# bbye98/mdhelper

Hardware: AMD Instinct MI355X
Metric: pair-distances binned/sec (higher is better)
Workload: dtype f32 filter + f64 contract arithmetic, u64 counts

## Files before the change

include/mdx.h:

```cpp
#ifndef MDX_H
#define MDX_H

#include <stddef.h>
#include <stdint.h>

#ifdef __cplusplus
extern "C" {
#endif

#define MDX_VERSION 100

#define MDX_OK 0
#define MDX_ERR_INVALID_VALUE (-1)
#define MDX_ERR_UNSUPPORTED (-2)
#define MDX_ERR_NO_DEVICE (-3)
#define MDX_ERR_HIP (-4)
#define MDX_ERR_ROCFFT (-5)
#define MDX_ERR_RCCL (-6)
#define MDX_ERR_OUT_OF_MEMORY (-7)
#define MDX_ERR_STATE (-8)
#define MDX_ERR_IO (-9)


const char *mdx_last_error(void);
// ... 39 lines not shown
#define MDX_RDF_ALGO_FILTER_F32 2
#define MDX_RDF_ALGO_CELL 3

int mdx_rdf_create(mdx_rdf_t *out, int dev, int n_bins, const double *edges,
                   int64_t excl1, int64_t excl2, int algo);
int mdx_rdf_destroy(mdx_rdf_t h);
int mdx_rdf_reset(mdx_rdf_t h);
int mdx_rdf_accumulate(mdx_rdf_t h, const float *pos1, int64_t n1, const float *pos2,
                       int64_t n2, const float *boxes, int64_t n_frames);
int mdx_rdf_set_drop_axis(mdx_rdf_t h, int axis);
int mdx_rdf_set_grouping(mdx_rdf_t h, int which, int64_t n_groups, const int64_t *offsets,
                         const double *masses);
int mdx_rdf_accumulate_device(mdx_rdf_t h, const float *d_pos1, int64_t n1,
                              const float *d_pos2, int64_t n2, const float *d_boxes,
                              int64_t n_frames);
int mdx_rdf_counts(mdx_rdf_t h, int64_t *counts);
int mdx_rdf_synchronize(mdx_rdf_t h);
int mdx_rdf_allreduce(mdx_rdf_t h, mdx_comm_t comm);
int mdx_rdf_stats(mdx_rdf_t h, int64_t *launches, double *kernel_ms,
                  int64_t *pairs_evaluated, int64_t *pairs_exact, int64_t *pairs_computed);
int mdx_rdf_enable_timing(mdx_rdf_t h, int on);
int mdx_rdf_debug_counters(mdx_rdf_t h, int64_t out[4]);
int mdx_rdf_kernel_clock(mdx_rdf_t h, double *hz);
int mdx_rdf_debug_sorted(mdx_rdf_t h, int64_t frame, int64_t n_pad, float *pw, float *po);

int mdx_radial_histogram(int dev, const float *pos1, int64_t n1, const float *pos2,
                         int64_t n2, int n_bins, const double *edges, const float dims[6],
                         int64_t excl1, int64_t excl2, int64_t *counts);

typedef struct mdx_sq *mdx_sq_t;

int mdx_sq_create(mdx_sq_t *out, int dev, const double *wavevectors, int64_t n_q,
                  const int64_t *group_offsets, int n_groups, const int32_t *pairs,
                  int n_pairs);
int mdx_sq_destroy(mdx_sq_t h);
int mdx_sq_reset(mdx_sq_t h);
int mdx_sq_set_grouping(mdx_sq_t h, int64_t n_molecules, const int64_t *offsets, const double *masses);
int mdx_sq_set_chains(mdx_sq_t h, int64_t chain_length);
int mdx_sq_accumulate(mdx_sq_t h, const float *pos, int64_t n, int64_t n_frames);
int mdx_sq_accumulate_device(mdx_sq_t h, const float *d_pos, int64_t n, int64_t n_frames);
int mdx_sq_synchronize(mdx_sq_t h);
int mdx_sq_result(mdx_sq_t h, double *ssf);
int mdx_sq_allreduce(mdx_sq_t h, mdx_comm_t comm);
int mdx_sq_stats(mdx_sq_t h, int64_t *launches, double *kernel_ms);
int mdx_sq_enable_timing(mdx_sq_t h, int on);
int mdx_fourier_sum(int dev, const double *wavevectors, int64_t n_q, const double *positions,
// ... 195 lines not shown
```

mdhelper_amd/_core.py:

```python

from __future__ import annotations

import ctypes
from ctypes import byref, c_double, c_int, c_int64, c_size_t, c_void_p

import numpy as np

from . import _lib
from ._lib import check, lib


def _ptr(a):
    return None if a is None else a.ctypes.data_as(c_void_p)


class DeviceArray:

    def __init__(self, shape, dtype, dev: int = 0):
        self.shape = tuple(int(s) for s in np.atleast_1d(shape))
        self.dtype = np.dtype(dtype)
        self.dev = dev
        self.nbytes = int(np.prod(self.shape)) * self.dtype.itemsize
        p = c_void_p()
        check(lib().mdx_malloc(dev, self.nbytes, byref(p)))
# ... 235 lines not shown
                                            _ptr(i1), n1, _ptr(i2), n2))

    def counts(self):
        out = np.zeros(self.n_bins, dtype=np.int64)
        check(lib().mdx_rdf_counts(self.handle, _ptr(out)))
        return out

    def synchronize(self):
        check(lib().mdx_rdf_synchronize(self.handle))

    def reset(self):
        check(lib().mdx_rdf_reset(self.handle))

    def allreduce(self, comm: RcclComm):
        check(lib().mdx_rdf_allreduce(self.handle, comm.handle))

    def stats(self):
        n, ms, pe, px, pc = c_int64(), c_double(), c_int64(), c_int64(), c_int64()
        check(lib().mdx_rdf_stats(self.handle, byref(n), byref(ms), byref(pe), byref(px), byref(pc)))
        raw = np.zeros(4, dtype=np.int64)
        check(lib().mdx_rdf_debug_counters(self.handle, _ptr(raw)))
        hz = c_double()
        check(lib().mdx_rdf_kernel_clock(self.handle, byref(hz)))
        return {"launches": n.value, "kernel_ms": ms.value, "pairs_evaluated": pe.value,
                "pairs_exact": px.value, "pairs_computed": pc.value,
                "cell_units": int(raw[1]), "cell_units_general": int(raw[2]),
                "clock_hz": hz.value}


def radial_histogram_device(pos1, pos2, n_bins, edges, dims, exclusion=None, dev=0):
    p1 = np.ascontiguousarray(pos1, dtype=np.float32).reshape(-1, 3)
    p2 = np.ascontiguousarray(pos2, dtype=np.float32).reshape(-1, 3)
    box = None if dims is None else np.ascontiguousarray(dims, dtype=np.float32).reshape(6)
    edges = np.ascontiguousarray(edges, dtype=np.float64)
    e1, e2 = (0, 0) if exclusion is None else (int(exclusion[0]), int(exclusion[1]))
    counts = np.zeros(n_bins, dtype=np.int64)
    same = pos2 is pos1
    check(lib().mdx_radial_histogram(dev, _ptr(p1), p1.shape[0], _ptr(p1 if same else p2),
                                     p2.shape[0], n_bins, _ptr(edges), _ptr(box), e1, e2,
                                     _ptr(counts)))
    return counts


class SqEngine(_Engine):

    _destroy = "mdx_sq_destroy"

    def __init__(self, wavevectors, group_sizes, pairs, *, dev=0, timing=False):
        self.q = np.ascontiguousarray(wavevectors, dtype=np.float64).reshape(-1, 3)
        self.offsets = np.concatenate(([0], np.cumsum(group_sizes))).astype(np.int64)
# ... 809 lines not shown
```

mdhelper_amd/_lib.py:

```python

from __future__ import annotations

import ctypes
import os
import pathlib
from ctypes import POINTER, c_char_p, c_double, c_float, c_int, c_int32, c_int64, c_size_t, c_uint64, c_void_p

_PKG = pathlib.Path(__file__).resolve().parent
LIB_PATH = pathlib.Path(os.environ.get("MDX_LIBRARY", _PKG / "libmdx.so"))

MDX_OK = 0
_EXC = {
    -1: ValueError,
    -2: NotImplementedError,
    -3: RuntimeError,
    -4: RuntimeError,
    -5: RuntimeError,
    -6: RuntimeError,
    -7: MemoryError,
    -8: RuntimeError,
    -9: OSError,
}

RDF_ALGO = {"auto": 0, "exact": 1, "filter": 2, "cell": 3}
# ... 21 lines not shown
    "mdx_synth_random_walk_f64": (c_int, [c_int, _vp, c_int64, c_int64, POINTER(c_float), c_float, c_uint64]),
    "mdx_comm_unique_id": (c_int, [_vp]),
    "mdx_comm_init_rank": (c_int, [POINTER(_vp), c_int, _vp, c_int, c_int]),
    "mdx_comm_destroy": (c_int, [_vp]),
    "mdx_comm_count": (c_int, [_vp, POINTER(c_int), POINTER(c_int), POINTER(c_int)]),
    "mdx_comm_barrier": (c_int, [_vp]),
    "mdx_comm_allreduce_f64": (c_int, [_vp, _vp, c_int64, c_int]),
    "mdx_comm_allreduce_i64": (c_int, [_vp, _vp, c_int64]),
    "mdx_rdf_create": (c_int, [POINTER(_vp), c_int, c_int, _vp, c_int64, c_int64, c_int]),
    "mdx_rdf_destroy": (c_int, [_vp]),
    "mdx_rdf_reset": (c_int, [_vp]),
    "mdx_rdf_accumulate": (c_int, [_vp, _vp, c_int64, _vp, c_int64, _vp, c_int64]),
    "mdx_rdf_accumulate_device": (c_int, [_vp, _vp, c_int64, _vp, c_int64, _vp, c_int64]),
    "mdx_rdf_set_drop_axis": (c_int, [_vp, c_int]),
    "mdx_rdf_set_grouping": (c_int, [_vp, c_int, c_int64, _vp, _vp]),
    "mdx_rdf_counts": (c_int, [_vp, _vp]),
    "mdx_rdf_synchronize": (c_int, [_vp]),
    "mdx_rdf_allreduce": (c_int, [_vp, _vp]),
    "mdx_rdf_stats": (c_int, [_vp, POINTER(c_int64), POINTER(c_double), POINTER(c_int64), POINTER(c_int64),
                              POINTER(c_int64)]),
    "mdx_rdf_enable_timing": (c_int, [_vp, c_int]),
    "mdx_rdf_debug_counters": (c_int, [_vp, _vp]),
    "mdx_rdf_kernel_clock": (c_int, [_vp, POINTER(c_double)]),
    "mdx_rdf_debug_sorted": (c_int, [_vp, c_int64, c_int64, _vp, _vp]),
    "mdx_radial_histogram": (c_int, [c_int, _vp, c_int64, _vp, c_int64, c_int, _vp, _vp, c_int64, c_int64, _vp]),
    "mdx_sq_create": (c_int, [POINTER(_vp), c_int, _vp, c_int64, _vp, c_int, _vp, c_int]),
    "mdx_sq_destroy": (c_int, [_vp]),
    "mdx_sq_reset": (c_int, [_vp]),
    "mdx_sq_accumulate": (c_int, [_vp, _vp, c_int64, c_int64]),
    "mdx_sq_accumulate_device": (c_int, [_vp, _vp, c_int64, c_int64]),
    "mdx_sq_result": (c_int, [_vp, _vp]),
    "mdx_sq_allreduce": (c_int, [_vp, _vp]),
    "mdx_sq_stats": (c_int, [_vp, POINTER(c_int64), POINTER(c_double)]),
    "mdx_sq_enable_timing": (c_int, [_vp, c_int]),
    "mdx_fourier_sum": (c_int, [c_int, _vp, c_int64, _vp, c_int64, _vp]),
    "mdx_isf_create": (c_int, [POINTER(_vp), c_int, _vp, c_int64, _vp, c_int, _vp, c_int, c_int, c_int]),
    "mdx_isf_destroy": (c_int, [_vp]),
    "mdx_isf_reset": (c_int, [_vp]),
    "mdx_isf_accumulate": (c_int, [_vp, _vp, c_int64, c_int64]),
    "mdx_isf_result": (c_int, [_vp, _vp, _vp]),
    "mdx_isf_stats": (c_int, [_vp, POINTER(c_int64), POINTER(c_double), POINTER(c_int64)]),
    "mdx_isf_enable_timing": (c_int, [_vp, c_int]),
    "mdx_msd_create": (c_int, [POINTER(_vp), c_int, c_int64, c_int, c_int]),
    "mdx_msd_destroy": (c_int, [_vp]),
    "mdx_msd_reset": (c_int, [_vp]),
    "mdx_msd_n_fft": (c_int, [_vp, POINTER(c_int64)]),
# ... 235 lines not shown
```

mdhelper_amd/csrc/mdx_rdf.hip:

```cpp

#include "mdx_common.hpp"
#include "mdx_internal.hpp"
#include "mdx_molecules.hpp"
#include "mdx_rdf_device.hpp"
#include "mdx_rdf_cell.hpp"
#include "mdx_traj.hpp"

#include <cmath>

namespace mdx {


static double thresh_ge(double e)
{
    if (!(e > 0.0))
        return 0.0;
    double t = e * e;
    while (std::sqrt(t) >= e && t > 0.0)
        t = std::nextafter(t, 0.0);
    while (std::sqrt(t) < e)
        t = std::nextafter(t, INFINITY);
    return t;
}

static double thresh_gt(double e)
{
    if (e < 0.0)
        return 0.0;
    return thresh_ge(std::nextafter(e, INFINITY));
}
// ... 280 lines not shown
    std::vector<double> edges;
    std::vector<double> thresh;
    double t_lo = 0, t_hi = 0;
    int64_t excl1 = 0, excl2 = 0;
    int algo = MDX_RDF_ALGO_AUTO;
    int n_rep = 32;
    DeviceBuffer d_thresh, d_counts, d_total, d_pack1, d_pack2, d_misc, d_tri;
    DeviceBuffer d_stats;
    DeviceBuffer d_work;
    const void *occ_kernel = nullptr;
    size_t occ_lds = 0;
    int64_t occ_blocks_per_xcd = 1;
    size_t last_offset = 0;
    int64_t last_frames = 0, last_n_pad = 0;
    bool last_lazy = false;
    MoleculeStage grouping[2];
    int drop_axis = -1;
    DeviceBuffer d_drop[2], d_drop_box;
    DeviceBuffer d_stage1[2], d_stage2[2], d_boxes[2], d_index[2];
    DeviceBuffer d_rawslab[2];
    StagePipeline pipe;
    DeviceBuffer d_pw1, d_po1, d_bb1, d_pw2, d_po2, d_bb2;
    DeviceBuffer d_bb16_1, d_bb16_2;
    StreamTimer timer;
    int64_t pairs_evaluated = 0;
    int64_t pairs_bruteforce = 0;
    bool reduced_global = false;
};

static int launch_tiles(mdx_rdf *h, RdfArgs &a, int mode, int ipt, bool pbc, bool excl,
                        int64_t n_frames)
{
    const int T = 256 * ipt;
    size_t base = sizeof(float4) * T + sizeof(double) * (h->n_bins + 1);
    const size_t lds_budget = 64 * 1024;
    int n_hist = 4;
    while (n_hist > 1 && base + size_t(n_hist) * h->n_bins * 4 > lds_budget)
        n_hist >>= 1;
    size_t lds = base + size_t(n_hist) * h->n_bins * 4;
    const bool gh = lds > lds_budget;
    if (gh)
        lds = sizeof(float4) * T;
    a.n_hist = n_hist;
    a.chunk = a.self ? 4 : 8;
    void (*kern)(RdfArgs) = nullptr;
#define MDX_PICK(M, I, P, E) \
// ... 25 lines not shown
        hipLaunchKernelGGL(kern, grid, dim3(256), lds, h->stream, a);
    }
    h->timer.end(ev);
    MDX_HIP(hipGetLastError());
    return MDX_OK;
}

static int accumulate_cell(mdx_rdf *h, const float *d_pos1, int64_t n1, const float *d_pos2,
                           int64_t n2, const float *d_boxes, int64_t n_frames, bool self, bool excl,
                           const float *d_tri = nullptr)
{
    const bool tri = d_tri != nullptr;
    const int64_t n1p = ceil_div(n1, 128) * 128, n2p = ceil_div(n2, 128) * 128;
    constexpr int64_t CHUNK_BOX_BYTES = CELL_CHUNK >= 4 ? 32 / CELL_CHUNK : 0;
    const int64_t per_frame = (32 + 1 + CHUNK_BOX_BYTES) * (n1p + (self ? 0 : n2p));
    const char *slab_env = getenv("MDX_RDF_SLAB_BYTES");
    const int64_t slab_bytes = slab_env ? std::max<int64_t>(1, atoll(slab_env)) : (int64_t(5) << 29);
    int64_t slab = std::max<int64_t>(1, slab_bytes / per_frame);
    slab = std::min<int64_t>(slab, 32768);
    if (slab >= 256)
        slab -= slab % 256;
    slab = std::min<int64_t>(slab, n_frames);
    const bool lazy_orig = !tri && h->excl1 <= 1 && h->excl2 <= 1;
    const size_t e_p1 = size_t(n1p) * slab, e_b1 = size_t(n1p / 64) * 2 * slab;
    const size_t e_c1 = CELL_CHUNK >= 4 ? size_t(n1p / CELL_CHUNK) * 2 * slab : 16;
    const size_t e_p2 = size_t(n2p) * slab, e_b2 = size_t(n2p / 64) * 2 * slab;
    const size_t e_c2 = CELL_CHUNK >= 4 ? size_t(n2p / CELL_CHUNK) * 2 * slab : 16;
    MDX_TRY(h->d_pw1.ensure(16 * e_p1));
    if (!lazy_orig)
        MDX_TRY(h->d_po1.ensure(16 * e_p1));
    MDX_TRY(h->d_bb1.ensure(16 * e_b1));
    MDX_TRY(h->d_bb16_1.ensure(16 * e_c1));
    if (!self) {
        MDX_TRY(h->d_bb16_2.ensure(16 * e_c2));
        MDX_TRY(h->d_pw2.ensure(16 * e_p2));
        if (!lazy_orig)
            MDX_TRY(h->d_po2.ensure(16 * e_p2));
        MDX_TRY(h->d_bb2.ensure(16 * e_b2));
    }
    unsigned *d_misc = h->d_misc.as<unsigned>();
    if (!tri)
        hipLaunchKernelGGL(rdf_check_boxes_kernel, dim3((unsigned)ceil_div(n_frames, 256)), dim3(256),
                           0, h->stream, d_boxes, n_frames, d_misc + 1);

    size_t base = sizeof(float4) * 256 + sizeof(double) * (h->n_bins + 1);
    const size_t lds_budget = 64 * 1024;
    const size_t lds_six_blocks = 13 * 1024;
    int n_hist = 8;
    while (n_hist > 4 && base + size_t(n_hist) * cell_hist_stride(h->n_bins) * 4 > lds_six_blocks)
        n_hist >>= 1;
    while (n_hist > 1 && base + size_t(n_hist) * cell_hist_stride(h->n_bins) * 4 > lds_budget)
        n_hist >>= 1;
    size_t lds = base + size_t(n_hist) * cell_hist_stride(h->n_bins) * 4;
    const bool gh = lds > lds_budget;
    if (gh)
        lds = sizeof(float4) * 256;
    const bool lower = h->edges.front() > 0.0;
    void (*kern)(CellArgs) = nullptr;
#define MDX_CELL_PICK(E, L)                                                                     \
    kern = tri ? (gh ? rdf_cell_pair_kernel<E, L, 1, true> : rdf_cell_pair_kernel<E, L, 0, true>) \
               : (gh ? rdf_cell_pair_kernel<E, L, 1> : rdf_cell_pair_kernel<E, L, 0>)
    if (excl && lower) MDX_CELL_PICK(true, true);
    else if (excl) MDX_CELL_PICK(true, false);
    else if (lower) MDX_CELL_PICK(false, true);
    else MDX_CELL_PICK(false, false);
#undef MDX_CELL_PICK
    if (h->occ_kernel != reinterpret_cast<const void *>(kern) || h->occ_lds != lds) {
        int per_cu = 0, cus = 0;
        MDX_HIP(hipOccupancyMaxActiveBlocksPerMultiprocessor(&per_cu, reinterpret_cast<const void *>(kern), 256, lds));
        MDX_HIP(hipDeviceGetAttribute(&cus, hipDeviceAttributeMultiprocessorCount, h->dev));
        h->occ_kernel = reinterpret_cast<const void *>(kern);
        h->occ_lds = lds;
        h->occ_blocks_per_xcd = std::max<int64_t>(1, int64_t(std::max(per_cu, 1)) * std::max(cus, 8) / 8);
    }
    const int64_t blocks_per_xcd = h->occ_blocks_per_xcd;

    hipStream_t s_sort = h->stream;
    for (int64_t f0 = 0; f0 < n_frames; f0 += slab) {
        const int64_t nf = std::min(slab, n_frames - f0);
        float4 *pw1 = h->d_pw1.as<float4>();
        float4 *po1 = lazy_orig ? nullptr : h->d_po1.as<float4>();
        float4 *bb1 = h->d_bb1.as<float4>(), *bc1 = h->d_bb16_1.as<float4>();
        float4 *pw2 = self ? pw1 : h->d_pw2.as<float4>();
        float4 *po2 = self ? po1 : (lazy_orig ? nullptr : h->d_po2.as<float4>());
        float4 *bb2 = self ? bb1 : h->d_bb2.as<float4>();
        float4 *bc2 = self ? bc1 : h->d_bb16_2.as<float4>();
        unsigned *d_maxabs = d_misc;
        h->last_offset = 0;
        h->last_frames = nf;
        h->last_n_pad = n1p;
        h->last_lazy = lazy_orig;
        {
            auto sort = tri ? rdf_cell_sort_kernel<true> : rdf_cell_sort_kernel<false>;
            const float *cells = tri ? d_tri + f0 * 9 : d_boxes + f0 * 6;
            hipLaunchKernelGGL(sort, dim3((unsigned)nf), dim3(SORT_THREADS), 0, s_sort,
                               d_pos1 + f0 * n1 * 3, cells, (int)n1, (int)n1p, excl ? h->excl1 : 0,
                               pw1, po1, bb1, bc1, d_maxabs);
            if (!self)
                hipLaunchKernelGGL(sort, dim3((unsigned)nf), dim3(SORT_THREADS), 0, s_sort,
                                   d_pos2 + f0 * n2 * 3, cells, (int)n2, (int)n2p,
                                   excl ? h->excl2 : 0, pw2, po2, bb2, bc2, d_maxabs);
        }
        CellArgs a{};
        a.pw1 = pw1;
        a.po1 = po1;
        a.bb1 = bb1;
        a.pw2 = pw2;
        a.po2 = po2;
        a.bb2 = bb2;
        a.bb16_2 = bc2;
        a.in1 = lazy_orig ? d_pos1 + f0 * n1 * 3 : nullptr;
        a.in2 = lazy_orig ? d_pos2 + f0 * n2 * 3 : nullptr;
        a.n1_in = (int)n1;
        a.n2_in = (int)n2;
        a.tags_everywhere = (self && h->excl1 == 1 && h->excl2 == 1) ? 0 : 1;
        a.boxes = tri ? nullptr : d_boxes + f0 * 6;
        a.tri = tri ? d_tri + f0 * 9 : nullptr;
        a.thresh = h->d_thresh.as<double>();
        a.counts = h->d_counts.as<unsigned long long>();
        a.maxabs_bits = d_maxabs;
        a.exact_counter = h->d_stats.as<unsigned long long>();
        a.tilepair_counter = a.exact_counter + 1;
        a.clock_counter = h->timer.enabled ? a.exact_counter + 3 : nullptr;
        a.t_lo = h->t_lo;
        a.t_hi = h->t_hi;
        a.r0 = h->edges.front();
        a.r1 = h->edges.back();
        a.n1p = (int)n1p;
        a.n2p = (int)n2p;
        a.n_bins = h->n_bins;
        a.n_hist = n_hist;
        a.n_rep = h->n_rep;
        a.self = self ? 1 : 0;
        a.work = h->d_work.as<unsigned>();
        {
            const char *fu = getenv("MDX_RDF_LDS_FLUSH_UNITS");
            a.flush_units = fu ? (unsigned)std::min<long long>(std::max<long long>(atoll(fu), 1), 1 << 18) : (1u << 18);
        }
        const int64_t tiles = n1p / 128;
        hipEvent_t ev = h->timer.begin();
        const int64_t launch_frames = std::max<int64_t>(8, std::min<int64_t>(32768, ((int64_t(1) << 30) / tiles) * 8));
        for (int64_t g0 = 0; g0 < nf; g0 += launch_frames) {
            a.frame0 = (int)g0;
            a.n_frames = (int)std::min<int64_t>(launch_frames, nf - g0);
            a.spread = a.n_frames < 8 ? 1 : 0;
            const int64_t items_per_xcd = a.spread ? ceil_div(int64_t(a.n_frames) * tiles, 8)
                                                   : ceil_div(a.n_frames, 8) * tiles;
            const unsigned grid = 8u * (unsigned)std::min<int64_t>(blocks_per_xcd, items_per_xcd);
            MDX_HIP(hipMemsetAsync(h->d_work.ptr, 0, CELL_WORK_BYTES, h->stream));
            hipLaunchKernelGGL(kern, dim3(grid), dim3(256), lds, h->stream, a);
        }
        h->timer.end(ev);
        MDX_HIP(hipGetLastError());
    }
    h->pairs_evaluated += n_frames * n1 * n2;
    return MDX_OK;
}

static int accumulate_ortho(mdx_rdf *h, const float *d_pos1, int64_t n1, const float *d_pos2,
                            int64_t n2, const float *d_boxes, int64_t n_frames)
{
    if (n_frames == 0 || n1 == 0 || n2 == 0)
        return MDX_OK;
    if (h->reduced_global)
        return fail(MDX_ERR_STATE, "handle holds all-reduced counts; call mdx_rdf_reset() first");
    const bool same = (d_pos2 == nullptr || (d_pos2 == d_pos1 && n2 == n1));
    if (d_pos2 == nullptr) {
        d_pos2 = d_pos1;
        n2 = n1;
    }
    const bool excl = h->excl1 > 0;
    const bool self = same && (!excl || h->excl1 == h->excl2);
    MDX_REQUIRE(n1 < (int64_t(1) << 30) && n2 < (int64_t(1) << 30), "too many particles");

    int algo = h->algo;
    if (algo == MDX_RDF_ALGO_AUTO)
        algo = d_boxes ? MDX_RDF_ALGO_CELL : MDX_RDF_ALGO_FILTER_F32;
// ... 389 lines not shown
        if (hipMemcpy(h->d_thresh.ptr, h->thresh.data(), sizeof(double) * (n_bins + 1),
                      hipMemcpyHostToDevice) != hipSuccess) {
            rc = fail(MDX_ERR_HIP, "threshold upload failed");
            break;
        }
    } while (0);
    if (rc != MDX_OK) {
        mdx_rdf_destroy(h);
        return rc;
    }
    *out = h;
    return mdx_rdf_reset(h);
}

int mdx_rdf_destroy(mdx_rdf_t h)
{
    if (!h)
        return MDX_OK;
    (void)hipSetDevice(h->dev);
    if (h->stream)
        (void)hipStreamSynchronize(h->stream);
    if (h->pipe.copy_stream)
        (void)hipStreamSynchronize(h->pipe.copy_stream);
    h->timer.destroy();
    h->pipe.destroy();
    for (DeviceBuffer *b : {&h->d_thresh, &h->d_counts, &h->d_total, &h->d_pack1, &h->d_pack2,
                            &h->d_stage1[0], &h->d_stage2[0], &h->d_boxes[0], &h->d_stage1[1],
                            &h->d_stage2[1], &h->d_boxes[1], &h->d_rawslab[0], &h->d_rawslab[1], &h->d_index[0], &h->d_index[1], &h->d_tri, &h->d_misc, &h->d_stats, &h->d_work, &h->d_pw1,
                            &h->d_po1, &h->d_bb1, &h->d_pw2, &h->d_po2, &h->d_bb2, &h->d_bb16_1,
                            &h->d_bb16_2, &h->d_drop[0], &h->d_drop[1], &h->d_drop_box})
        b->recycle();
    h->grouping[0].recycle();
    h->grouping[1].recycle();
    if (h->stream)
        stream_release(h->stream);
    delete h;
    return MDX_OK;
}

int mdx_rdf_reset(mdx_rdf_t h)
{
    MDX_REQUIRE(h, "NULL handle");
    MDX_TRY(set_device(h->dev));
    MDX_HIP(hipStreamSynchronize(h->stream));
    MDX_HIP(hipMemsetAsync(h->d_counts.ptr, 0, sizeof(uint64_t) * size_t(h->n_rep) * h->n_bins,
                           h->stream));
    MDX_HIP(hipMemsetAsync(h->d_misc.ptr, 0, 64, h->stream));
    MDX_HIP(hipMemsetAsync(h->d_stats.ptr, 0, RDF_STAT_BYTES, h->stream));
    MDX_HIP(hipStreamSynchronize(h->stream));
    h->timer.reset();
    h->pairs_evaluated = 0;
    h->pairs_bruteforce = 0;
    h->reduced_global = false;
    return MDX_OK;
}

int mdx_rdf_set_drop_axis(mdx_rdf_t h, int axis)
{
    MDX_REQUIRE(h, "NULL handle");
    MDX_REQUIRE(axis >= -1 && axis <= 2, "axis must be 0, 1, 2 or -1 (none)");
    h->drop_axis = axis;
    return MDX_OK;
}

int mdx_rdf_set_grouping(mdx_rdf_t h, int which, int64_t n_groups, const int64_t *offsets,
                         const double *masses)
{
    MDX_REQUIRE(h, "NULL handle");
    MDX_REQUIRE(which == 1 || which == 2, "which must be 1 or 2");
    MDX_TRY(set_device(h->dev));
    MDX_HIP(hipStreamSynchronize(h->stream));
    return h->grouping[which - 1].set(n_groups, offsets, masses);
}

int mdx_rdf_accumulate_device(mdx_rdf_t h, const float *d_pos1, int64_t n1, const float *d_pos2,
// ... 153 lines not shown
int mdx_rdf_kernel_clock(mdx_rdf_t h, double *hz)
{
    MDX_REQUIRE(h && hz, "NULL argument");
    MDX_TRY(set_device(h->dev));
    unsigned long long st[5];
    MDX_TRY(read_stats(h, st));
    *hz = st[4] ? double(st[3]) / double(st[4]) * 1.0e8 : 0.0;
    return MDX_OK;
}

int mdx_rdf_debug_counters(mdx_rdf_t h, int64_t out[4])
{
    MDX_REQUIRE(h && out, "NULL argument");
    MDX_TRY(set_device(h->dev));
    unsigned long long raw[5];
    MDX_TRY(read_stats(h, raw));
    out[0] = (int64_t)raw[0];
    out[1] = (int64_t)raw[1];
    out[2] = (int64_t)raw[2];
    out[3] = h->pairs_bruteforce;
    return MDX_OK;
}

int mdx_rdf_debug_sorted(mdx_rdf_t h, int64_t frame, int64_t n_pad, float *pw, float *po)
{
    MDX_REQUIRE(h && pw && po, "NULL argument");
    MDX_TRY(set_device(h->dev));
    MDX_HIP(hipStreamSynchronize(h->stream));
    MDX_REQUIRE(h->last_frames > 0, "no slab has gone through the cell-sorted path yet");
    MDX_REQUIRE(frame >= 0 && frame < h->last_frames, "frame %lld outside the last slab (%lld frames)",
                (long long)frame, (long long)h->last_frames);
    MDX_REQUIRE(n_pad == h->last_n_pad, "n_pad is %lld for the last slab", (long long)h->last_n_pad);
    MDX_HIP(hipMemcpy(pw, h->d_pw1.as<float4>() + h->last_offset + frame * n_pad, size_t(16) * n_pad,
                      hipMemcpyDeviceToHost));
    if (h->last_lazy)
        return fail(MDX_ERR_STATE, "the last slab has no sorted originals (exclusion 0 or 1): pw is filled, "
                    "po is not; MDX_RDF_SORTED_ORIGINALS=1 materialises them");
    MDX_HIP(hipMemcpy(po, h->d_po1.as<float4>() + h->last_offset + frame * n_pad, size_t(16) * n_pad,
                      hipMemcpyDeviceToHost));
    return MDX_OK;
}

int mdx_rdf_enable_timing(mdx_rdf_t h, int on)
{
    MDX_REQUIRE(h, "NULL handle");
    h->timer.enabled = on != 0;
// ... 40 lines not shown
```

mdhelper_amd/csrc/mdx_rdf_cell.hpp:

```cpp
#pragma once

#include "mdx_rdf_device.hpp"

struct CellArgs {
    const float4 *pw1, *po1, *bb1;
    const float4 *pw2, *po2, *bb2;
    const float4 *bb16_2;
    const float *in1, *in2;
    int n1_in, n2_in;
    const float *boxes;
    const float *tri;
    const double *thresh;
    unsigned long long *counts;
    const unsigned *maxabs_bits;
    unsigned long long *exact_counter;
    unsigned long long *tilepair_counter;
    unsigned long long *clock_counter;
    double t_lo, t_hi, r0, r1;
    int n1p, n2p;
    int n_bins, n_hist, n_rep;
    int self, frame0;
    int n_frames;
    int tags_everywhere;
    unsigned *work;
// ... 81 lines not shown
#pragma unroll
        for (int k = 2; k >= 0; --k) {
            const double s = floor(r[k] / B[4 * k]);
#pragma unroll
            for (int c = 0; c <= k; ++c)
                r[c] -= s * B[3 * k + c];
        }
        wx = (float)r[0];
        wy = (float)r[1];
        wz = (float)r[2];
    }
    __device__ inline void cell(float wx, float wy, float wz, const int *nc, int &cx, int &cy,
                                int &cz) const
    {
        const double sz = (double)wz / B[8];
        const double sy = ((double)wy - sz * B[7]) / B[4];
        const double sx = ((double)wx - sy * B[3] - sz * B[6]) / B[0];
        cx = min(max((int)floor(sx * nc[0]), 0), nc[0] - 1);
        cy = min(max((int)floor(sy * nc[1]), 0), nc[1] - 1);
        cz = min(max((int)floor(sz * nc[2]), 0), nc[2] - 1);
    }
};

template <bool TRI>
__global__ __launch_bounds__(SORT_THREADS) void rdf_cell_sort_kernel(
    const float *__restrict__ pos, const float *__restrict__ boxes, int n, int n_pad, int64_t excl,
    float4 *__restrict__ pw, float4 *__restrict__ po, float4 *__restrict__ bb,
    float4 *__restrict__ bb16, unsigned *maxabs_bits)
{
    __shared__ unsigned cnt[CELL_MAX];
    __shared__ unsigned part[SORT_THREADS];
    const int tid = threadIdx.x;
    const int frame = blockIdx.x;
    const float *P = pos + int64_t(frame) * n * 3;
    float4 *PW = pw + int64_t(frame) * n_pad;
    float4 *PO = po + int64_t(frame) * n_pad;
    CellGrid g;
    TriCell tc;
    if (TRI) {
        tc.init(boxes + int64_t(frame) * 9);
        const float hb[3] = {(float)tc.h[0], (float)tc.h[1], (float)tc.h[2]};
        g.init(hb, n);
    } else {
        g.init(boxes + int64_t(frame) * 6, n);
    }
    const int ncell = g.n_cells();
// ... 64 lines not shown
        float wx, wy, wz;
        if (TRI) {
            tc.wrap(x, y, z, wx, wy, wz);
            tc.cell(wx, wy, wz, g.nc, cx, cy, cz);
            x = wx, y = wy, z = wz;
        } else {
            wx = g.wrap(x, 0, cx), wy = g.wrap(y, 1, cy), wz = g.wrap(z, 2, cz);
        }
        unsigned slot = atomicAdd(&cnt[g.key(cx, cy, cz)], 1u);
        float tag = __int_as_float(excl > 0 ? int(int64_t(a) / excl) : a);
        PW[slot] = make_float4(wx, wy, wz, tag);
        if (po)
            PO[slot] = make_float4(x, y, z, tag);
    }
    const float qnan = __int_as_float(0x7fc00000);
    for (int a = n + tid; a < n_pad; a += SORT_THREADS) {
        PW[a] = make_float4(qnan, qnan, qnan, __int_as_float(-1));
        if (po)
            PO[a] = make_float4(qnan, qnan, qnan, __int_as_float(-1));
    }
    __threadfence_block();
    __syncthreads();

    const int lane = tid & 63, wave = tid >> 6;
    const int n_tiles = n_pad / 64;
    float4 *BB = bb + int64_t(frame) * n_tiles * 2;
    float4 *BB16 = bb16 + int64_t(frame) * n_tiles * 2 * CELL_NCHUNK;
#pragma unroll 2
    for (int t = wave; t < n_tiles; t += SORT_THREADS / 64) {
        float4 v = PW[t * 64 + lane];
        const float inf = __int_as_float(0x7f800000);
        bool ok = v.x == v.x;
        float lo[3] = {ok ? v.x : inf, ok ? v.y : inf, ok ? v.z : inf};
        float hi[3] = {ok ? v.x : -inf, ok ? v.y : -inf, ok ? v.z : -inf};
        for (int off = 1; off < 64; off <<= 1) {
#pragma unroll
            for (int k = 0; k < 3; ++k) {
                lo[k] = fminf(lo[k], __shfl_xor(lo[k], off));
                hi[k] = fmaxf(hi[k], __shfl_xor(hi[k], off));
            }
            if (CELL_CHUNK >= 4 && off == CELL_CHUNK / 2 && (lane & (CELL_CHUNK - 1)) == 0) {
                const int c = t * CELL_NCHUNK + lane / CELL_CHUNK;
                BB16[c * 2] = make_float4(lo[0], lo[1], lo[2], 0.f);
                BB16[c * 2 + 1] = make_float4(hi[0], hi[1], hi[2], 0.f);
            }
        }
        if (lane == 0) {
            BB[2 * t] = make_float4(lo[0], lo[1], lo[2], 0.f);
            BB[2 * t + 1] = make_float4(hi[0], hi[1], hi[2], 0.f);
        }
    }
}

__device__ inline double rdf_rsq_contract_tri(const float *Bf, const float4 &pi, const float4 &pj)
{
    const double b00 = Bf[0], b10 = Bf[3], b11 = Bf[4], b20 = Bf[6], b21 = Bf[7], b22 = Bf[8];
    const double dx = (double)(pj.x - pi.x), dy = (double)(pj.y - pi.y), dz = (double)(pj.z - pi.z);
    double best = 1.0e300;
#pragma unroll 1
    for (int ix = -1; ix < 2; ++ix) {
        const double rx = dx + b00 * (double)ix;
#pragma unroll 1
        for (int iy = -1; iy < 2; ++iy) {
            const double ry0 = rx + b10 * (double)iy;
            const double ry1 = dy + b11 * (double)iy;
#pragma unroll 1
            for (int iz = -1; iz < 2; ++iz) {
                const double rz0 = ry0 + b20 * (double)iz;
                const double rz1 = ry1 + b21 * (double)iz;
                const double rz2 = dz + b22 * (double)iz;
                const double dsq = (rz0 * rz0 + rz1 * rz1) + rz2 * rz2;
                best = dsq < best ? dsq : best;
            }
        }
// ... 747 lines not shown
```

Before: 2115 billion.

## Overlap next-slab cell sort on a side stream with current histogram kernel

Splits frames into slabs with double-buffered sorted-position sets and sorts the next slab on a side stream while the main stream runs the cell histogram kernel on the current slab. The histogram grid is shrunk to leave holes for the sort blocks. It adds a compact, grid-strided sort kernel with 16-bit packed cell counters and smaller first slabs to shorten pipeline fill. This hides sort latency at the cost of extra device memory, event synchronisation, and a slightly smaller histogram grid.

After: 2156 billion, median of 6. +2.0%, better.

```diff
diff --git a/include/mdx.h b/include/mdx.h
--- a/include/mdx.h
+++ b/include/mdx.h
@@ -85,6 +85,7 @@
 int mdx_rdf_enable_timing(mdx_rdf_t h, int on);
 int mdx_rdf_debug_counters(mdx_rdf_t h, int64_t out[4]);
 int mdx_rdf_kernel_clock(mdx_rdf_t h, double *hz);
+int mdx_rdf_slabs_sorted_beside(mdx_rdf_t h, int64_t *out);
 int mdx_rdf_debug_sorted(mdx_rdf_t h, int64_t frame, int64_t n_pad, float *pw, float *po);
 
 int mdx_radial_histogram(int dev, const float *pos1, int64_t n1, const float *pos2,
diff --git a/mdhelper_amd/_core.py b/mdhelper_amd/_core.py
--- a/mdhelper_amd/_core.py
+++ b/mdhelper_amd/_core.py
@@ -281,10 +281,12 @@
         check(lib().mdx_rdf_debug_counters(self.handle, _ptr(raw)))
         hz = c_double()
         check(lib().mdx_rdf_kernel_clock(self.handle, byref(hz)))
+        beside = c_int64()
+        check(lib().mdx_rdf_slabs_sorted_beside(self.handle, byref(beside)))
         return {"launches": n.value, "kernel_ms": ms.value, "pairs_evaluated": pe.value,
                 "pairs_exact": px.value, "pairs_computed": pc.value,
                 "cell_units": int(raw[1]), "cell_units_general": int(raw[2]),
-                "clock_hz": hz.value}
+                "slabs_sorted_beside": beside.value, "clock_hz": hz.value}
 
 
 def radial_histogram_device(pos1, pos2, n_bins, edges, dims, exclusion=None, dev=0):
diff --git a/mdhelper_amd/_lib.py b/mdhelper_amd/_lib.py
--- a/mdhelper_amd/_lib.py
+++ b/mdhelper_amd/_lib.py
@@ -67,6 +67,7 @@
     "mdx_rdf_enable_timing": (c_int, [_vp, c_int]),
     "mdx_rdf_debug_counters": (c_int, [_vp, _vp]),
     "mdx_rdf_kernel_clock": (c_int, [_vp, POINTER(c_double)]),
+    "mdx_rdf_slabs_sorted_beside": (c_int, [_vp, POINTER(c_int64)]),
     "mdx_rdf_debug_sorted": (c_int, [_vp, c_int64, c_int64, _vp, _vp]),
     "mdx_radial_histogram": (c_int, [c_int, _vp, c_int64, _vp, c_int64, c_int, _vp, _vp, c_int64, c_int64, _vp]),
     "mdx_sq_create": (c_int, [POINTER(_vp), c_int, _vp, c_int64, _vp, c_int, _vp, c_int]),
diff --git a/mdhelper_amd/csrc/mdx_rdf.hip b/mdhelper_amd/csrc/mdx_rdf.hip
--- a/mdhelper_amd/csrc/mdx_rdf.hip
+++ b/mdhelper_amd/csrc/mdx_rdf.hip
@@ -6,6 +6,7 @@
 #include "mdx_rdf_cell.hpp"
 #include "mdx_traj.hpp"
 
+#include <cstring>
 #include <cmath>
 
 namespace mdx {
@@ -332,6 +333,14 @@
     StagePipeline pipe;
     DeviceBuffer d_pw1, d_po1, d_bb1, d_pw2, d_po2, d_bb2;
     DeviceBuffer d_bb16_1, d_bb16_2;
+    hipStream_t side = nullptr;
+    hipEvent_t ev_fork = nullptr;
+    hipEvent_t ev_sorted[2] = {nullptr, nullptr};
+    hipEvent_t ev_read[2] = {nullptr, nullptr};
+    hipEvent_t ev_join = nullptr;
+    int64_t slabs_sorted_beside = 0;
+    size_t occ_static_lds = 0;
+    int occ_per_cu = 1;
     StreamTimer timer;
     int64_t pairs_evaluated = 0;
     int64_t pairs_bruteforce = 0;
@@ -403,22 +412,6 @@
         slab -= slab % 256;
     slab = std::min<int64_t>(slab, n_frames);
     const bool lazy_orig = !tri && h->excl1 <= 1 && h->excl2 <= 1;
-    const size_t e_p1 = size_t(n1p) * slab, e_b1 = size_t(n1p / 64) * 2 * slab;
-    const size_t e_c1 = CELL_CHUNK >= 4 ? size_t(n1p / CELL_CHUNK) * 2 * slab : 16;
-    const size_t e_p2 = size_t(n2p) * slab, e_b2 = size_t(n2p / 64) * 2 * slab;
-    const size_t e_c2 = CELL_CHUNK >= 4 ? size_t(n2p / CELL_CHUNK) * 2 * slab : 16;
-    MDX_TRY(h->d_pw1.ensure(16 * e_p1));
-    if (!lazy_orig)
-        MDX_TRY(h->d_po1.ensure(16 * e_p1));
-    MDX_TRY(h->d_bb1.ensure(16 * e_b1));
-    MDX_TRY(h->d_bb16_1.ensure(16 * e_c1));
-    if (!self) {
-        MDX_TRY(h->d_bb16_2.ensure(16 * e_c2));
-        MDX_TRY(h->d_pw2.ensure(16 * e_p2));
-        if (!lazy_orig)
-            MDX_TRY(h->d_po2.ensure(16 * e_p2));
-        MDX_TRY(h->d_bb2.ensure(16 * e_b2));
-    }
     unsigned *d_misc = h->d_misc.as<unsigned>();
     if (!tri)
         hipLaunchKernelGGL(rdf_check_boxes_kernel, dim3((unsigned)ceil_div(n_frames, 256)), dim3(256),
@@ -448,92 +441,204 @@
 #undef MDX_CELL_PICK
     if (h->occ_kernel != reinterpret_cast<const void *>(kern) || h->occ_lds != lds) {
         int per_cu = 0, cus = 0;
+        hipFuncAttributes fa{};
         MDX_HIP(hipOccupancyMaxActiveBlocksPerMultiprocessor(&per_cu, reinterpret_cast<const void *>(kern), 256, lds));
         MDX_HIP(hipDeviceGetAttribute(&cus, hipDeviceAttributeMultiprocessorCount, h->dev));
+        MDX_HIP(hipFuncGetAttributes(&fa, reinterpret_cast<const void *>(kern)));
         h->occ_kernel = reinterpret_cast<const void *>(kern);
         h->occ_lds = lds;
+        h->occ_static_lds = fa.sharedSizeBytes;
+        h->occ_per_cu = std::max(per_cu, 1);
         h->occ_blocks_per_xcd = std::max<int64_t>(1, int64_t(std::max(per_cu, 1)) * std::max(cus, 8) / 8);
     }
     const int64_t blocks_per_xcd = h->occ_blocks_per_xcd;
 
-    hipStream_t s_sort = h->stream;
-    for (int64_t f0 = 0; f0 < n_frames; f0 += slab) {
-        const int64_t nf = std::min(slab, n_frames - f0);
-        float4 *pw1 = h->d_pw1.as<float4>();
-        float4 *po1 = lazy_orig ? nullptr : h->d_po1.as<float4>();
-        float4 *bb1 = h->d_bb1.as<float4>(), *bc1 = h->d_bb16_1.as<float4>();
-        float4 *pw2 = self ? pw1 : h->d_pw2.as<float4>();
-        float4 *po2 = self ? po1 : (lazy_orig ? nullptr : h->d_po2.as<float4>());
-        float4 *bb2 = self ? bb1 : h->d_bb2.as<float4>();
-        float4 *bc2 = self ? bc1 : h->d_bb16_2.as<float4>();
-        unsigned *d_maxabs = d_misc;
-        h->last_offset = 0;
-        h->last_frames = nf;
-        h->last_n_pad = n1p;
-        h->last_lazy = lazy_orig;
-        {
-            auto sort = tri ? rdf_cell_sort_kernel<true> : rdf_cell_sort_kernel<false>;
-            const float *cells = tri ? d_tri + f0 * 9 : d_boxes + f0 * 6;
-            hipLaunchKernelGGL(sort, dim3((unsigned)nf), dim3(SORT_THREADS), 0, s_sort,
-                               d_pos1 + f0 * n1 * 3, cells, (int)n1, (int)n1p, excl ? h->excl1 : 0,
-                               pw1, po1, bb1, bc1, d_maxabs);
+    constexpr int64_t S0 = 16;
+    const char *sb_env = getenv("MDX_RDF_SORT_BESIDE");
+    const size_t sort_small_lds = sort_small_lds_bytes();
+    const size_t cu_lds = size_t(160) * 1024;
+    bool beside = !tri && !(sb_env && strcmp(sb_env, "0") == 0) && n_frames > slab && n1 <= SORT_SMALL_MAX_N &&
+                  n2 <= SORT_SMALL_MAX_N && blocks_per_xcd >= 2 &&
+                  size_t(h->occ_per_cu - 1) * (h->occ_static_lds + lds) + sort_small_lds <= cu_lds;
+    if (beside && !h->ev_join) {
+        if (!h->side)
+            MDX_TRY(stream_acquire(&h->side));
+        for (hipEvent_t *e : {&h->ev_fork, &h->ev_sorted[0], &h->ev_sorted[1], &h->ev_read[0], &h->ev_read[1], &h->ev_join})
+            if (!*e)
+                MDX_HIP(hipEventCreateWithFlags(e, hipEventDisableTiming));
+    }
+
+    const size_t e_p1 = size_t(n1p) * slab, e_b1 = size_t(n1p / 64) * 2 * slab;
+    const size_t e_c1 = CELL_CHUNK >= 4 ? size_t(n1p / CELL_CHUNK) * 2 * slab : 16;
+    const size_t e_p2 = size_t(n2p) * slab, e_b2 = size_t(n2p / 64) * 2 * slab;
+    const size_t e_c2 = CELL_CHUNK >= 4 ? size_t(n2p / CELL_CHUNK) * 2 * slab : 16;
+    auto ensure_sets = [&](size_t n_sets) -> int {
+        MDX_TRY(h->d_pw1.ensure(16 * e_p1 * n_sets));
+        if (!lazy_orig)
+            MDX_TRY(h->d_po1.ensure(16 * e_p1 * n_sets));
+        MDX_TRY(h->d_bb1.ensure(16 * e_b1 * n_sets));
+        MDX_TRY(h->d_bb16_1.ensure(16 * e_c1 * n_sets));
+        if (!self) {
+            MDX_TRY(h->d_bb16_2.ensure(16 * e_c2 * n_sets));
+            MDX_TRY(h->d_pw2.ensure(16 * e_p2 * n_sets));
+            if (!lazy_orig)
+                MDX_TRY(h->d_po2.ensure(16 * e_p2 * n_sets));
+            MDX_TRY(h->d_bb2.ensure(16 * e_b2 * n_sets));
+        }
+        return MDX_OK;
+    };
+    if (beside && ensure_sets(2) == MDX_ERR_OUT_OF_MEMORY)
+        beside = false;
+    MDX_TRY(ensure_sets(beside ? 2 : 1));
+    std::vector<int64_t> lens;
+    for (int64_t f0 = 0; f0 < n_frames;) {
+        int64_t step = slab;
+        if (beside && slab >= 8 && lens.size() < 2) {
+            step = slab >> (2 - lens.size());
+            if (step >= 256)
+                step -= step % 256;
+        }
+        step = std::min(step, n_frames - f0);
+        lens.push_back(step);
+        f0 += step;
+    }
+    unsigned *d_maxabs = d_misc;
+
+    struct Set {
+        float4 *pw1, *po1, *bb1, *bc1, *pw2, *po2, *bb2, *bc2;
+    };
+    auto set_of = [&](int b) {
+        Set s;
+        s.pw1 = h->d_pw1.as<float4>() + b * e_p1;
+        s.po1 = lazy_orig ? nullptr : h->d_po1.as<float4>() + b * e_p1;
+        s.bb1 = h->d_bb1.as<float4>() + b * e_b1;
+        s.bc1 = h->d_bb16_1.as<float4>() + b * e_c1;
+        s.pw2 = self ? s.pw1 : h->d_pw2.as<float4>() + b * e_p2;
+        s.po2 = self ? s.po1 : (lazy_orig ? nullptr : h->d_po2.as<float4>() + b * e_p2);
+        s.bb2 = self ? s.bb1 : h->d_bb2.as<float4>() + b * e_b2;
+        s.bc2 = self ? s.bc1 : h->d_bb16_2.as<float4>() + b * e_c2;
+        return s;
+    };
+    auto launch_sort = [&](const Set &s, int64_t f0, int64_t nf, hipStream_t stream, unsigned small_grid) {
+        const float *cells = tri ? d_tri + f0 * 9 : d_boxes + f0 * 6;
+        if (small_grid) {
+            auto sort = rdf_cell_sort_small_kernel<SORT_SMALL_THREADS>;
+            hipLaunchKernelGGL(sort, dim3(small_grid), dim3(SORT_SMALL_THREADS), sort_small_lds, stream, d_pos1 + f0 * n1 * 3,
+                               cells, (int)n1, (int)n1p, excl ? h->excl1 : 0, s.pw1, s.po1, s.bb1, s.bc1, d_maxabs,
+                               (int)nf);
             if (!self)
-                hipLaunchKernelGGL(sort, dim3((unsigned)nf), dim3(SORT_THREADS), 0, s_sort,
-                                   d_pos2 + f0 * n2 * 3, cells, (int)n2, (int)n2p,
-                                   excl ? h->excl2 : 0, pw2, po2, bb2, bc2, d_maxabs);
+                hipLaunchKernelGGL(sort, dim3(small_grid), dim3(SORT_SMALL_THREADS), sort_small_lds, stream,
+                                   d_pos2 + f0 * n2 * 3, cells, (int)n2, (int)n2p, excl ? h->excl2 : 0, s.pw2,
+                                   s.po2, s.bb2, s.bc2, d_maxabs, (int)nf);
+            return;
         }
-        CellArgs a{};
-        a.pw1 = pw1;
-        a.po1 = po1;
-        a.bb1 = bb1;
-        a.pw2 = pw2;
-        a.po2 = po2;
-        a.bb2 = bb2;
-        a.bb16_2 = bc2;
-        a.in1 = lazy_orig ? d_pos1 + f0 * n1 * 3 : nullptr;
-        a.in2 = lazy_orig ? d_pos2 + f0 * n2 * 3 : nullptr;
-        a.n1_in = (int)n1;
-        a.n2_in = (int)n2;
-        a.tags_everywhere = (self && h->excl1 == 1 && h->excl2 == 1) ? 0 : 1;
-        a.boxes = tri ? nullptr : d_boxes + f0 * 6;
-        a.tri = tri ? d_tri + f0 * 9 : nullptr;
-        a.thresh = h->d_thresh.as<double>();
-        a.counts = h->d_counts.as<unsigned long long>();
-        a.maxabs_bits = d_maxabs;
-        a.exact_counter = h->d_stats.as<unsigned long long>();
-        a.tilepair_counter = a.exact_counter + 1;
-        a.clock_counter = h->timer.enabled ? a.exact_counter + 3 : nullptr;
-        a.t_lo = h->t_lo;
-        a.t_hi = h->t_hi;
-        a.r0 = h->edges.front();
-        a.r1 = h->edges.back();
-        a.n1p = (int)n1p;
-        a.n2p = (int)n2p;
-        a.n_bins = h->n_bins;
-        a.n_hist = n_hist;
-        a.n_rep = h->n_rep;
-        a.self = self ? 1 : 0;
-        a.work = h->d_work.as<unsigned>();
-        {
-            const char *fu = getenv("MDX_RDF_LDS_FLUSH_UNITS");
-            a.flush_units = fu ? (unsigned)std::min<long long>(std::max<long long>(atoll(fu), 1), 1 << 18) : (1u << 18);
+        auto sort = tri ? rdf_cell_sort_kernel<true> : rdf_cell_sort_kernel<false>;
+        hipLaunchKernelGGL(sort, dim3((unsigned)nf), dim3(SORT_THREADS), 0, stream, d_pos1 + f0 * n1 * 3, cells,
+                           (int)n1, (int)n1p, excl ? h->excl1 : 0, s.pw1, s.po1, s.bb1, s.bc1, d_maxabs);
+        if (!self)
+            hipLaunchKernelGGL(sort, dim3((unsigned)nf), dim3(SORT_THREADS), 0, stream, d_pos2 + f0 * n2 * 3,
+                               cells, (int)n2, (int)n2p, excl ? h->excl2 : 0, s.pw2, s.po2, s.bb2, s.bc2,
+                               d_maxabs);
+    };
+
+    auto slabs = [&]() -> int {
+        int64_t f0 = 0;
+        for (size_t k = 0; k < lens.size(); f0 += lens[k], ++k) {
+            const int64_t nf = lens[k];
+            const int b = beside ? int(k & 1) : 0;
+            const Set s = set_of(b);
+            h->last_offset = b * e_p1;
+            h->last_frames = nf;
+            h->last_n_pad = n1p;
+            h->last_lazy = lazy_orig;
+            if (!beside || k == 0)
+                launch_sort(s, f0, nf, h->stream, 0);
+            else
+                MDX_HIP(hipStreamWaitEvent(h->stream, h->ev_sorted[b], 0));
+            int64_t holes = 0;
+            if (beside && k + 1 < lens.size()) {
+                const int64_t nf_next = lens[k + 1];
+                holes = ceil_div(ceil_div(S0 * nf_next, nf), 8) * 8;
+                holes = std::min<int64_t>(holes, 8 * (blocks_per_xcd / 2));
+                if (k > 0)
+                    MDX_HIP(hipStreamWaitEvent(h->side, h->ev_read[b ^ 1], 0));
+                launch_sort(set_of(b ^ 1), f0 + nf, nf_next, h->side, (unsigned)std::min<int64_t>(holes, nf_next));
+                MDX_HIP(hipEventRecord(h->ev_sorted[b ^ 1], h->side));
+                h->slabs_sorted_beside += 1;
+            }
+            CellArgs a{};
+            a.pw1 = s.pw1;
+            a.po1 = s.po1;
+            a.bb1 = s.bb1;
+            a.pw2 = s.pw2;
+            a.po2 = s.po2;
+            a.bb2 = s.bb2;
+            a.bb16_2 = s.bc2;
+            a.in1 = lazy_orig ? d_pos1 + f0 * n1 * 3 : nullptr;
+            a.in2 = lazy_orig ? d_pos2 + f0 * n2 * 3 : nullptr;
+            a.n1_in = (int)n1;
+            a.n2_in = (int)n2;
+            a.tags_everywhere = (self && h->excl1 == 1 && h->excl2 == 1) ? 0 : 1;
+            a.boxes = tri ? nullptr : d_boxes + f0 * 6;
+            a.tri = tri ? d_tri + f0 * 9 : nullptr;
+            a.thresh = h->d_thresh.as<double>();
+            a.counts = h->d_counts.as<unsigned long long>();
+            a.maxabs_bits = d_maxabs;
+            a.exact_counter = h->d_stats.as<unsigned long long>();
+            a.tilepair_counter = a.exact_counter + 1;
+            a.clock_counter = h->timer.enabled ? a.exact_counter + 3 : nullptr;
+            a.t_lo = h->t_lo;
+            a.t_hi = h->t_hi;
+            a.r0 = h->edges.front();
+            a.r1 = h->edges.back();
+            a.n1p = (int)n1p;
+            a.n2p = (int)n2p;
+            a.n_bins = h->n_bins;
+            a.n_hist = n_hist;
+            a.n_rep = h->n_rep;
+            a.self = self ? 1 : 0;
+            a.work = h->d_work.as<unsigned>();
+            {
+                const char *fu = getenv("MDX_RDF_LDS_FLUSH_UNITS");
+                a.flush_units = fu ? (unsigned)std::min<long long>(std::max<long long>(atoll(fu), 1), 1 << 18) : (1u << 18);
+            }
+            const int64_t tiles = n1p / 128;
+            hipEvent_t ev = h->timer.begin();
+            const int64_t launch_frames = std::max<int64_t>(8, std::min<int64_t>(32768, ((int64_t(1) << 30) / tiles) * 8));
+            for (int64_t g0 = 0; g0 < nf; g0 += launch_frames) {
+                a.frame0 = (int)g0;
+                a.n_frames = (int)std::min<int64_t>(launch_frames, nf - g0);
+                a.spread = a.n_frames < 8 ? 1 : 0;
+                const int64_t items_per_xcd = a.spread ? ceil_div(int64_t(a.n_frames) * tiles, 8)
+                                                       : ceil_div(a.n_frames, 8) * tiles;
+                const unsigned grid = 8u * (unsigned)std::min<int64_t>(blocks_per_xcd - holes / 8, items_per_xcd);
+                MDX_HIP(hipMemsetAsync(h->d_work.ptr, 0, CELL_WORK_BYTES, h->stream));
+                hipLaunchKernelGGL(kern, dim3(grid), dim3(256), lds, h->stream, a);
+            }
+            h->timer.end(ev);
+            MDX_HIP(hipGetLastError());
+            if (beside)
+                MDX_HIP(hipEventRecord(h->ev_read[b], h->stream));
         }
-        const int64_t tiles = n1p / 128;
-        hipEvent_t ev = h->timer.begin();
-        const int64_t launch_frames = std::max<int64_t>(8, std::min<int64_t>(32768, ((int64_t(1) << 30) / tiles) * 8));
-        for (int64_t g0 = 0; g0 < nf; g0 += launch_frames) {
-            a.frame0 = (int)g0;
-            a.n_frames = (int)std::min<int64_t>(launch_frames, nf - g0);
-            a.spread = a.n_frames < 8 ? 1 : 0;
-            const int64_t items_per_xcd = a.spread ? ceil_div(int64_t(a.n_frames) * tiles, 8)
-                                                   : ceil_div(a.n_frames, 8) * tiles;
-            const unsigned grid = 8u * (unsigned)std::min<int64_t>(blocks_per_xcd, items_per_xcd);
-            MDX_HIP(hipMemsetAsync(h->d_work.ptr, 0, CELL_WORK_BYTES, h->stream));
-            hipLaunchKernelGGL(kern, dim3(grid), dim3(256), lds, h->stream, a);
+        return MDX_OK;
+    };
+    int rc = MDX_OK;
+    if (beside) {
+        MDX_HIP(hipEventRecord(h->ev_fork, h->stream));
+        MDX_HIP(hipStreamWaitEvent(h->side, h->ev_fork, 0));
+        rc = slabs();
+        hipError_t e = hipEventRecord(h->ev_join, h->side);
+        if (e == hipSuccess)
+            e = hipStreamWaitEvent(h->stream, h->ev_join, 0);
+        if (e != hipSuccess) {
+            (void)hipStreamSynchronize(h->side);
+            if (rc == MDX_OK)
+                rc = fail(MDX_ERR_HIP, "joining the sort stream failed: %s", hipGetErrorString(e));
         }
-        h->timer.end(ev);
-        MDX_HIP(hipGetLastError());
-    }
+    } else {
+        rc = slabs();
+    }
+    MDX_TRY(rc);
     h->pairs_evaluated += n_frames * n1 * n2;
     return MDX_OK;
 }
@@ -969,8 +1074,13 @@
         (void)hipStreamSynchronize(h->stream);
     if (h->pipe.copy_stream)
         (void)hipStreamSynchronize(h->pipe.copy_stream);
+    if (h->side)
+        (void)hipStreamSynchronize(h->side);
     h->timer.destroy();
     h->pipe.destroy();
+    for (hipEvent_t e : {h->ev_fork, h->ev_join, h->ev_sorted[0], h->ev_sorted[1], h->ev_read[0], h->ev_read[1]})
+        if (e)
+            (void)hipEventDestroy(e);
     for (DeviceBuffer *b : {&h->d_thresh, &h->d_counts, &h->d_total, &h->d_pack1, &h->d_pack2,
                             &h->d_stage1[0], &h->d_stage2[0], &h->d_boxes[0], &h->d_stage1[1],
                             &h->d_stage2[1], &h->d_boxes[1], &h->d_rawslab[0], &h->d_rawslab[1], &h->d_index[0], &h->d_index[1], &h->d_tri, &h->d_misc, &h->d_stats, &h->d_work, &h->d_pw1,
@@ -979,6 +1089,8 @@
         b->recycle();
     h->grouping[0].recycle();
     h->grouping[1].recycle();
+    if (h->side)
+        stream_release(h->side);
     if (h->stream)
         stream_release(h->stream);
     delete h;
@@ -998,6 +1110,7 @@
     h->timer.reset();
     h->pairs_evaluated = 0;
     h->pairs_bruteforce = 0;
+    h->slabs_sorted_beside = 0;
     h->reduced_global = false;
     return MDX_OK;
 }
@@ -1197,6 +1310,13 @@
     return MDX_OK;
 }
 
+int mdx_rdf_slabs_sorted_beside(mdx_rdf_t h, int64_t *out)
+{
+    MDX_REQUIRE(h && out, "NULL argument");
+    *out = h->slabs_sorted_beside;
+    return MDX_OK;
+}
+
 int mdx_rdf_debug_sorted(mdx_rdf_t h, int64_t frame, int64_t n_pad, float *pw, float *po)
 {
     MDX_REQUIRE(h && pw && po, "NULL argument");
diff --git a/mdhelper_amd/csrc/mdx_rdf_cell.hpp b/mdhelper_amd/csrc/mdx_rdf_cell.hpp
--- a/mdhelper_amd/csrc/mdx_rdf_cell.hpp
+++ b/mdhelper_amd/csrc/mdx_rdf_cell.hpp
@@ -127,6 +127,39 @@
     }
 };
 
+template <int THREADS>
+__device__ inline void cell_tile_boxes(const float4 *PW, float4 *bb, float4 *bb16, int frame, int n_pad, int tid)
+{
+    const int lane = tid & 63, wave = tid >> 6;
+    const int n_tiles = n_pad / 64;
+    float4 *BB = bb + int64_t(frame) * n_tiles * 2;
+    float4 *BB16 = bb16 + int64_t(frame) * n_tiles * 2 * CELL_NCHUNK;
+#pragma unroll 2
+    for (int t = wave; t < n_tiles; t += THREADS / 64) {
+        float4 v = PW[t * 64 + lane];
+        const float inf = __int_as_float(0x7f800000);
+        bool ok = v.x == v.x;
+        float lo[3] = {ok ? v.x : inf, ok ? v.y : inf, ok ? v.z : inf};
+        float hi[3] = {ok ? v.x : -inf, ok ? v.y : -inf, ok ? v.z : -inf};
+        for (int off = 1; off < 64; off <<= 1) {
+#pragma unroll
+            for (int k = 0; k < 3; ++k) {
+                lo[k] = fminf(lo[k], __shfl_xor(lo[k], off));
+                hi[k] = fmaxf(hi[k], __shfl_xor(hi[k], off));
+            }
+            if (CELL_CHUNK >= 4 && off == CELL_CHUNK / 2 && (lane & (CELL_CHUNK - 1)) == 0) {
+                const int c = t * CELL_NCHUNK + lane / CELL_CHUNK;
+                BB16[c * 2] = make_float4(lo[0], lo[1], lo[2], 0.f);
+                BB16[c * 2 + 1] = make_float4(hi[0], hi[1], hi[2], 0.f);
+            }
+        }
+        if (lane == 0) {
+            BB[2 * t] = make_float4(lo[0], lo[1], lo[2], 0.f);
+            BB[2 * t + 1] = make_float4(hi[0], hi[1], hi[2], 0.f);
+        }
+    }
+}
+
 template <bool TRI>
 __global__ __launch_bounds__(SORT_THREADS) void rdf_cell_sort_kernel(
     const float *__restrict__ pos, const float *__restrict__ boxes, int n, int n_pad, int64_t excl,
@@ -237,34 +270,141 @@
     __threadfence_block();
     __syncthreads();
 
-    const int lane = tid & 63, wave = tid >> 6;
-    const int n_tiles = n_pad / 64;
-    float4 *BB = bb + int64_t(frame) * n_tiles * 2;
-    float4 *BB16 = bb16 + int64_t(frame) * n_tiles * 2 * CELL_NCHUNK;
-#pragma unroll 2
-    for (int t = wave; t < n_tiles; t += SORT_THREADS / 64) {
-        float4 v = PW[t * 64 + lane];
-        const float inf = __int_as_float(0x7f800000);
-        bool ok = v.x == v.x;
-        float lo[3] = {ok ? v.x : inf, ok ? v.y : inf, ok ? v.z : inf};
-        float hi[3] = {ok ? v.x : -inf, ok ? v.y : -inf, ok ? v.z : -inf};
-        for (int off = 1; off < 64; off <<= 1) {
-#pragma unroll
-            for (int k = 0; k < 3; ++k) {
-                lo[k] = fminf(lo[k], __shfl_xor(lo[k], off));
-                hi[k] = fmaxf(hi[k], __shfl_xor(hi[k], off));
-            }
-            if (CELL_CHUNK >= 4 && off == CELL_CHUNK / 2 && (lane & (CELL_CHUNK - 1)) == 0) {
-                const int c = t * CELL_NCHUNK + lane / CELL_CHUNK;
-                BB16[c * 2] = make_float4(lo[0], lo[1], lo[2], 0.f);
-                BB16[c * 2 + 1] = make_float4(hi[0], hi[1], hi[2], 0.f);
-            }
-        }
-        if (lane == 0) {
-            BB[2 * t] = make_float4(lo[0], lo[1], lo[2], 0.f);
-            BB[2 * t + 1] = make_float4(hi[0], hi[1], hi[2], 0.f);
-        }
-    }
+    cell_tile_boxes<SORT_THREADS>(PW, bb, bb16, frame, n_pad, tid);
+}
+
+__device__ inline double cell_uniform_d(double v)
+{
+    return __hiloint2double(__builtin_amdgcn_readfirstlane(__double2hiint(v)),
+                            __builtin_amdgcn_readfirstlane(__double2loint(v)));
+}
+
+constexpr int SORT_SMALL_THREADS = 256;
+constexpr int SORT_SMALL_BATCH = 8;
+constexpr int SORT_SMALL_BATCH_SCATTER = 4;
+constexpr int64_t SORT_SMALL_MAX_N = 65535;
+constexpr size_t sort_small_lds_bytes() { return size_t(4) * (CELL_MAX / 2 + SORT_SMALL_THREADS); }
+template <int THREADS>
+__global__ __launch_bounds__(THREADS, 7) void rdf_cell_sort_small_kernel(
+    const float *__restrict__ pos, const float *__restrict__ boxes, int n, int n_pad, int64_t excl,
+    float4 *__restrict__ pw, float4 *__restrict__ po, float4 *__restrict__ bb,
+    float4 *__restrict__ bb16, unsigned *maxabs_bits, int nf)
+{
+    extern __shared__ __align__(16) unsigned sort_small_lds[];
+    unsigned *cnt = sort_small_lds;
+    unsigned *part = sort_small_lds + CELL_MAX / 2;
+    const int tid = threadIdx.x;
+    const unsigned excl32 = (unsigned)min(excl, (int64_t)0x7fffffff);
+    float m = 0.0f;
+    for (int frame = blockIdx.x; frame < nf; frame += gridDim.x) {
+        const float *P = pos + int64_t(frame) * n * 3;
+        float4 *PW = pw + int64_t(frame) * n_pad;
+        float4 *PO = po + int64_t(frame) * n_pad;
+        CellGrid g;
+        g.init(boxes + int64_t(frame) * 6, n);
+#pragma unroll
+        for (int k = 0; k < 3; ++k) {
+            g.Ld[k] = cell_uniform_d(g.Ld[k]);
+            g.invLd[k] = cell_uniform_d(g.invLd[k]);
+            g.nc[k] = __builtin_amdgcn_readfirstlane(g.nc[k]);
+        }
+        const int ncell = g.n_cells();
+        for (int c = tid; c < (ncell + 1) / 2; c += THREADS)
+            cnt[c] = 0u;
+        __syncthreads();
+
+        for (int a0 = tid; a0 < n; a0 += THREADS * SORT_SMALL_BATCH) {
+            float x[SORT_SMALL_BATCH], y[SORT_SMALL_BATCH], z[SORT_SMALL_BATCH];
+#pragma unroll
+            for (int u = 0; u < SORT_SMALL_BATCH; ++u) {
+                const int a = min(a0 + u * THREADS, n - 1);
+                x[u] = P[3 * a], y[u] = P[3 * a + 1], z[u] = P[3 * a + 2];
+            }
+#pragma unroll
+            for (int u = 0; u < SORT_SMALL_BATCH; ++u)
+                asm volatile("" : "+v"(x[u]), "+v"(y[u]), "+v"(z[u]));
+#pragma unroll
+            for (int u = 0; u < SORT_SMALL_BATCH; ++u) {
+                if (a0 + u * THREADS >= n)
+                    break;
+                int cx, cy, cz;
+                g.wrap(x[u], 0, cx);
+                g.wrap(y[u], 1, cy);
+                g.wrap(z[u], 2, cz);
+                const int c = g.key(cx, cy, cz);
+                atomicAdd(&cnt[c >> 1], 1u << (16 * (c & 1)));
+                float am = fmaxf(fabsf(x[u]), fmaxf(fabsf(y[u]), fabsf(z[u])));
+                m = fmaxf(m, am == am ? am : __int_as_float(0x7f800000));
+            }
+        }
+        __syncthreads();
+
+        const int per = (((ncell + 1) / 2 + THREADS - 1) / THREADS);
+        const int nw = (ncell + 1) / 2;
+        const int w0 = min(tid * per, nw), w1 = min(w0 + per, nw);
+        unsigned local = 0;
+        for (int w = w0; w < w1; ++w) {
+            const unsigned v = cnt[w];
+            local += (v & 0xffffu) + (v >> 16);
+        }
+        part[tid] = local;
+        __syncthreads();
+        for (int off = 1; off < THREADS; off <<= 1) {
+            unsigned v = (tid >= off) ? part[tid - off] : 0u;
+            __syncthreads();
+            part[tid] += v;
+            __syncthreads();
+        }
+        unsigned run = part[tid] - local;
+        for (int w = w0; w < w1; ++w) {
+            const unsigned v = cnt[w];
+            const unsigned lo = run, hi = run + (v & 0xffffu);
+            cnt[w] = lo | (hi << 16);
+            run = hi + (v >> 16);
+        }
+        __syncthreads();
+
+        for (int a0 = tid; a0 < n; a0 += THREADS * SORT_SMALL_BATCH_SCATTER) {
+            float x[SORT_SMALL_BATCH_SCATTER], y[SORT_SMALL_BATCH_SCATTER], z[SORT_SMALL_BATCH_SCATTER];
+#pragma unroll
+            for (int u = 0; u < SORT_SMALL_BATCH_SCATTER; ++u) {
+                const int a = min(a0 + u * THREADS, n - 1);
+                x[u] = P[3 * a], y[u] = P[3 * a + 1], z[u] = P[3 * a + 2];
+            }
+#pragma unroll
+            for (int u = 0; u < SORT_SMALL_BATCH_SCATTER; ++u)
+                asm volatile("" : "+v"(x[u]), "+v"(y[u]), "+v"(z[u]));
+#pragma unroll
+            for (int u = 0; u < SORT_SMALL_BATCH_SCATTER; ++u) {
+                const int a = a0 + u * THREADS;
+                if (a >= n)
+                    break;
+                int cx, cy, cz;
+                const float wx = g.wrap(x[u], 0, cx), wy = g.wrap(y[u], 1, cy), wz = g.wrap(z[u], 2, cz);
+                const int c = g.key(cx, cy, cz);
+                const int sh = 16 * (c & 1);
+                const unsigned slot = (atomicAdd(&cnt[c >> 1], 1u << sh) >> sh) & 0xffffu;
+                float tag = __int_as_float(excl > 0 ? int(unsigned(a) / excl32) : a);
+                PW[slot] = make_float4(wx, wy, wz, tag);
+                if (po)
+                    PO[slot] = make_float4(x[u], y[u], z[u], tag);
+            }
+        }
+        const float qnan = __int_as_float(0x7fc00000);
+        for (int a = n + tid; a < n_pad; a += THREADS) {
+            PW[a] = make_float4(qnan, qnan, qnan, __int_as_float(-1));
+            if (po)
+                PO[a] = make_float4(qnan, qnan, qnan, __int_as_float(-1));
+        }
+        __threadfence_block();
+        __syncthreads();
+        cell_tile_boxes<THREADS>(PW, bb, bb16, frame, n_pad, tid);
+    }
+    unsigned bits = __float_as_uint(m);
+    for (int off = 32; off > 0; off >>= 1)
+        bits = max(bits, (unsigned)__shfl_xor((int)bits, off));
+    if ((tid & 63) == 0 && bits)
+        atomicMax(maxabs_bits, bits);
 }
 
 __device__ inline double rdf_rsq_contract_tri(const float *Bf, const float4 &pi, const float4 &pj)
```
